# jaehyuck0103/OpenMAVIS

Measured on AMD Instinct MI355X. Metric: multi-cam frames/sec (ORB extract+match) + LocalBA iters/sec, 5x720x540, higher is better.
Workload: dtype u8

## Files before the change

openmavis_amd/csrc/omv_device.h:

```cpp
#pragma once
#include <hip/hip_runtime.h>
#include <stdint.h>

namespace omv {

__device__ __forceinline__ int round_even(float v) { return (int)__builtin_rintf(v); }

__device__ __forceinline__ float fast_atan2_deg(float y, float x) {
    const float r2d = (float)(180.0 / 3.14159265358979323846);
    const float k1 = 0.9997878412794807f * r2d;
    const float k3 = -0.3258083974640975f * r2d;
    const float k5 = 0.1555786518463281f * r2d;
    const float k7 = -0.04432655554792128f * r2d;
    const float eps = (float)2.220446049250313080847e-16;
    float ax = __builtin_fabsf(x), ay = __builtin_fabsf(y), a, c, c2;
    if (ax >= ay) {
        c = ay / (ax + eps);
        c2 = c * c;
        a = (((k7 * c2 + k5) * c2 + k3) * c2 + k1) * c;
    } else {
        c = ax / (ay + eps);
        c2 = c * c;
        a = 90.f - (((k7 * c2 + k5) * c2 + k3) * c2 + k1) * c;
    }
// ... 180 lines not shown
    w = x + r;
    if (ix >= 0x3f2ca140) {
        v = (float)iy;
        return (float)(1 - ((hx >> 30) & 2)) * (v - 2.0f * (x - (w * w / (w + v) - r)));
    }
    if (iy == 1) return w;
    float a, t;
    z = __uint_as_float(f32_bits(w) & 0xfffff000u);
    v = r - (z - x);
    t = a = -1.0f / w;
    t = __uint_as_float(f32_bits(t) & 0xfffff000u);
    s = 1.0f + t * z;
    return t + a * (s + t * v);
}
__device__ inline float glibc_tanf(float x) {
    const int32_t ix = (int32_t)(f32_bits(x) & 0x7fffffffu);
    if (ix <= 0x3f490fda) return glibc_kernel_tanf(x, 0.0f, 1);
    const double xd = (double)x, nd = rint(xd * 0.6366197723675814);
    const int n = (int)nd;
    const double r = xd - nd * 1.5707963267948966;
    const float y0 = (float)r, y1 = (float)(r - (double)y0);
    return glibc_kernel_tanf(y0, y1, 1 - ((n & 1) << 1));
}

__device__ __forceinline__ int xcd_block(int n_logical) {
    const int chunk = (n_logical + 7) >> 3;
    const int b = (int)(blockIdx.x & 7) * chunk + (int)(blockIdx.x >> 3);
    return b < n_logical ? b : -1;
}
__host__ inline int xcd_grid(int n_logical) { return (n_logical + 7) & ~7; }

}
extern "C" __device__ __attribute__((const)) uint32_t omv_llvm_mul_u24(uint32_t, uint32_t) __asm("llvm.amdgcn.mul.u24.i32");
namespace omv {
__device__ __forceinline__ int mul_u24(int a, int b) { return (int)omv_llvm_mul_u24((uint32_t)a, (uint32_t)b); }

struct MatcherKnobs {
    int bow_top = -1, tri_slices = -1, tri_ecap = -1, tri_walk_seq = 0;
    int cand_mode = 0;
    int cand_pw = -1;
};
MatcherKnobs matcher_knobs(const struct ::omv_matcher *m);
size_t matcher_kf_entry_cap(const struct ::omv_matcher *m);

}
```

openmavis_amd/csrc/orb_extract.hip:

```cpp
#include <hip/hip_runtime.h>

#include <algorithm>
#include <cmath>
#include <cstdlib>
#include <climits>
#include <cstdio>
#include <cstring>
#include <vector>

#include "../../include/omv.h"
#include "omv_device.h"
#include "omv_host.h"
#include "omv_introsort.h"

namespace {

constexpr int kMaxLevels = 16;
constexpr int kOrbStages = 4;
constexpr int kEdge = 19;
constexpr int kMinB = kEdge - 3;
#define OMV_PATTERN_TABLE_BEGIN
#define OMV_PATTERN_TABLE_END
constexpr int kPattern[256 * 4] = {
#include "orb_pattern_31.inc"
// ... 28 lines not shown
    int xq_off, use_xq;
    uint32_t m_quads, m_groups, m_w;
};

struct Cell {
    int level, y0, y1, x0, x1;
};

struct Geom {
    int nlevels;
    int W, H;
    int ini_th, min_th;
    int n_cells;
    int cell_cap;
    long long pyr_bytes;
    long long cand_per_img;
    int out_per_img;
    int n_max;
    int node_cap;
    int ccnt_cap;
    unsigned long long umax_pk;
    LevelGeom lv[kMaxLevels];
};

struct XTab {
    int sx0, sx1, coef;
};

struct __attribute__((aligned(16))) XQuad {
    int a[2];
    uint32_t sel[4], cf[4];
    int pad[2];
};
static_assert(sizeof(XQuad) == 48, "XQuad LDS addressing");

__device__ __forceinline__ const uint8_t *level_base(const Geom &g, const uint8_t *images, size_t img_stride,
                                                     size_t pitch0, const uint8_t *pyr, int img, int l,
                                                     int *pitch) {
    if (l == 0) {
        *pitch = (int)pitch0;
        return images + (size_t)img * img_stride;
    }
    *pitch = g.lv[l].pitch;
    return pyr + (size_t)img * g.pyr_bytes + g.lv[l].off;
}

constexpr int kPyrBlock = 16;

__device__ __forceinline__ int vmix(int b0, int b1, int h0, int h1) {
    return ((omv::mul_u24(b0, h0 >> 4) >> 16) + (omv::mul_u24(b1, h1 >> 4) >> 16) + 2) >> 2;
}

__global__ void __launch_bounds__(256) pyr_resize_kernel(Geom g, int l, const uint8_t *images, size_t img_stride,
                                                         size_t pitch0, uint8_t *pyr, const XTab *xt,
                                                         const XTab *yt, const XQuad *xq, int n_images) {
    extern __shared__ __attribute__((aligned(16))) uint32_t pyr_lds[];
    const LevelGeom &L = g.lv[l];
    const int img = blockIdx.y, tid = threadIdx.x;
    const int dy0 = blockIdx.x * kPyrBlock, dy1 = min(dy0 + kPyrBlock, L.h);
    int sp;
    const uint8_t *src = level_base(g, images, img_stride, pitch0, pyr, img, l - 1, &sp);
    const int sw = g.lv[l - 1].w;
    const int ndw = ((sw + 15) >> 4) << 2;
    const int nq = (L.w + 3) >> 2;
    XTab *xs = reinterpret_cast<XTab *>(pyr_lds);
    XQuad *xqs = reinterpret_cast<XQuad *>(pyr_lds);
    uint32_t *rows = pyr_lds + 12 * nq;
    const int sy0 = yt[L.ytab_off + dy0].sx0, sy1 = yt[L.ytab_off + dy1 - 1].sx1;
    const int nr = sy1 - sy0 + 1;
    XTab *ys = reinterpret_cast<XTab *>(rows + nr * ndw + 4);
    const bool quad = L.use_xq != 0;
    if (quad)
        for (int i = tid; i < nq; i += 256) xqs[i] = xq[L.xq_off + i];
    else
        for (int i = tid; i < L.w; i += 256) xs[i] = xt[L.xtab_off + i];
    if (tid < dy1 - dy0) ys[tid] = yt[L.ytab_off + dy0 + tid];
    if ((sp & 15) == 0 && (((uintptr_t)src) & 15) == 0) {
        const int n4 = ndw >> 2;
        const uint32_t m4 = g.lv[l - 1].m_groups;
        for (int q = tid; q < nr * n4; q += 256) {
            const int r = (int)__umulhi((uint32_t)q, m4), i = q - r * n4;
            reinterpret_cast<uint4 *>(rows)[q] = reinterpret_cast<const uint4 *>(src + (size_t)(sy0 + r) * sp)[i];
        }
    } else {
        uint8_t *b = reinterpret_cast<uint8_t *>(rows);
        const uint32_t mw = g.lv[l - 1].m_w;
        for (int q = tid; q < nr * sw; q += 256) {
            const int r = (int)__umulhi((uint32_t)q, mw), i = q - r * sw;
            b[(size_t)r * ndw * 4 + i] = src[(size_t)(sy0 + r) * sp + i];
        }
    }
    __syncthreads();
    const uint32_t mq = L.m_quads;
    typedef unsigned short u16x2 __attribute__((ext_vector_type(2)));
    for (int q = tid; q < (dy1 - dy0) * nq; q += 256) {
        const int r = (int)__umulhi((uint32_t)q, mq), qd = q - omv::mul_u24(r, nq), dx0 = qd * 4,
                  dy = dy0 + r;
        const XTab y = ys[r];
        const int b0 = (short)(y.coef & 0xffff), b1 = (short)(y.coef >> 16);
        uint32_t packed = 0;
        if (quad) {
            const XQuad X = *reinterpret_cast<const XQuad *>(reinterpret_cast<const char *>(xqs) + omv::mul_u24(qd, 48u));
            const uint32_t *R0 = rows + omv::mul_u24(y.sx0 - sy0, ndw),
                           *R1 = rows + omv::mul_u24(y.sx1 - sy0, ndw);
            const uint32_t u0[4] = {R0[X.a[0]], R0[X.a[0] + 1], R0[X.a[1]], R0[X.a[1] + 1]};
            const uint32_t u1[4] = {R1[X.a[0]], R1[X.a[0] + 1], R1[X.a[1]], R1[X.a[1] + 1]};
#pragma unroll
            for (int j = 0; j < 4; ++j) {
                const int pp = 2 * (j >> 1);
                const u16x2 cf = __builtin_bit_cast(u16x2, X.cf[j]);
                const int h0 = (int)__builtin_amdgcn_udot2(
                    __builtin_bit_cast(u16x2, __builtin_amdgcn_perm(u0[pp + 1], u0[pp], X.sel[j])), cf, 0u, false);
                const int h1 = (int)__builtin_amdgcn_udot2(
                    __builtin_bit_cast(u16x2, __builtin_amdgcn_perm(u1[pp + 1], u1[pp], X.sel[j])), cf, 0u, false);
                packed |= (uint32_t)vmix(b0, b1, h0, h1) << (8 * j);
            }
        } else {
            const uint8_t *R0 = reinterpret_cast<const uint8_t *>(rows + omv::mul_u24(y.sx0 - sy0, ndw));
            const uint8_t *R1 = reinterpret_cast<const uint8_t *>(rows + omv::mul_u24(y.sx1 - sy0, ndw));
#pragma unroll
            for (int j = 0; j < 4; ++j) {
                const int dx = dx0 + j;
                if (dx < L.w) {
                    const XTab x = xs[dx];
                    const int a0 = (short)(x.coef & 0xffff), a1 = (short)(x.coef >> 16);
                    const int h0 = R0[x.sx0] * a0 + R0[x.sx1] * a1;
                    const int h1 = R1[x.sx0] * a0 + R1[x.sx1] * a1;
                    const int v = vmix(b0, b1, h0, h1);
                    packed |= (uint32_t)min(v, 255) << (8 * j);
                }
            }
        }
        uint8_t *dst = pyr + (size_t)img * g.pyr_bytes + L.off + (size_t)dy * L.pitch;
        if (dx0 + 3 < L.w) {
            *reinterpret_cast<uint32_t *>(dst + dx0) = packed;
        } else {
            for (int j = 0; j < 4 && dx0 + j < L.w; ++j) dst[dx0 + j] = (uint8_t)(packed >> (8 * j));
        }
    }
}


struct PyrBand {
    int own_lo, own_hi, need_lo, need_hi;
};
constexpr int kPyrChainMaxImages = 16;
__global__ void __launch_bounds__(256) pyr_chain_kernel(Geom g, const uint8_t *images, size_t img_stride, size_t pitch0,
                                                        uint8_t *pyr, const XTab *xt, const XTab *yt, const XQuad *xq,
                                                        const PyrBand *bands, int buf_dw, int tab_dw) {
    extern __shared__ __attribute__((aligned(16))) uint32_t pyr_lds[];
    const int b = blockIdx.x, img = blockIdx.y, tid = threadIdx.x;
    const PyrBand *B = bands + (size_t)b * kMaxLevels;
    uint32_t *prev = pyr_lds, *cur = pyr_lds + buf_dw;
    uint32_t *tab = pyr_lds + 2 * (size_t)buf_dw + 4;
    XTab *ys = reinterpret_cast<XTab *>(tab + tab_dw);
    XQuad *xqs = reinterpret_cast<XQuad *>(tab);
    XTab *xs = reinterpret_cast<XTab *>(tab);
    {
        const PyrBand b0 = B[0];
        const int sw = g.lv[0].w, ndw = ((sw + 15) >> 4) << 2, nr = b0.need_hi - b0.need_lo;
        const uint8_t *src = images + (size_t)img * img_stride;
        if ((pitch0 & 15) == 0 && (((uintptr_t)src) & 15) == 0) {
            const int n4 = ndw >> 2;
            const uint32_t m4 = g.lv[0].m_groups;
            for (int q = tid; q < nr * n4; q += 256) {
                const int r = (int)__umulhi((uint32_t)q, m4), i = q - r * n4;
                reinterpret_cast<uint4 *>(prev)[q] = reinterpret_cast<const uint4 *>(src + (size_t)(b0.need_lo + r) * pitch0)[i];
            }
        } else {
            uint8_t *bb = reinterpret_cast<uint8_t *>(prev);
            const uint32_t mw = g.lv[0].m_w;
            for (int q = tid; q < nr * sw; q += 256) {
                const int r = (int)__umulhi((uint32_t)q, mw), i = q - r * sw;
                bb[(size_t)r * ndw * 4 + i] = src[(size_t)(b0.need_lo + r) * pitch0 + i];
            }
        }
    }
    __syncthreads();
    typedef unsigned short u16x2 __attribute__((ext_vector_type(2)));
    for (int l = 1; l < g.nlevels; ++l) {
        const LevelGeom &L = g.lv[l];
        const PyrBand bp = B[l - 1], bc = B[l];
        const int sndw = ((g.lv[l - 1].w + 15) >> 4) << 2, cndw = ((L.w + 15) >> 4) << 2;
        const int nq = (L.w + 3) >> 2, nr = bc.need_hi - bc.need_lo;
        const bool quad = L.use_xq != 0;
        if (quad)
            for (int i = tid; i < nq; i += 256) xqs[i] = xq[L.xq_off + i];
        else
            for (int i = tid; i < L.w; i += 256) xs[i] = xt[L.xtab_off + i];
        for (int i = tid; i < nr; i += 256) ys[i] = yt[L.ytab_off + bc.need_lo + i];
        __syncthreads();
        const uint32_t mq = L.m_quads;
        for (int q = tid; q < nr * nq; q += 256) {
            const int r = (int)__umulhi((uint32_t)q, mq), qd = q - omv::mul_u24(r, nq), dx0 = qd * 4,
                      dy = bc.need_lo + r;
            const XTab y = ys[r];
            const int b0 = (short)(y.coef & 0xffff), b1 = (short)(y.coef >> 16);
            uint32_t packed = 0;
            if (quad) {
                const XQuad X = *reinterpret_cast<const XQuad *>(reinterpret_cast<const char *>(xqs) + omv::mul_u24(qd, 48u));
                const uint32_t *R0 = prev + omv::mul_u24(y.sx0 - bp.need_lo, sndw),
                               *R1 = prev + omv::mul_u24(y.sx1 - bp.need_lo, sndw);
                const uint32_t u0[4] = {R0[X.a[0]], R0[X.a[0] + 1], R0[X.a[1]], R0[X.a[1] + 1]};
                const uint32_t u1[4] = {R1[X.a[0]], R1[X.a[0] + 1], R1[X.a[1]], R1[X.a[1] + 1]};
#pragma unroll
                for (int j = 0; j < 4; ++j) {
                    const int pp = 2 * (j >> 1);
                    const u16x2 cf = __builtin_bit_cast(u16x2, X.cf[j]);
                    const int h0 = (int)__builtin_amdgcn_udot2(
                        __builtin_bit_cast(u16x2, __builtin_amdgcn_perm(u0[pp + 1], u0[pp], X.sel[j])), cf, 0u, false);
                    const int h1 = (int)__builtin_amdgcn_udot2(
                        __builtin_bit_cast(u16x2, __builtin_amdgcn_perm(u1[pp + 1], u1[pp], X.sel[j])), cf, 0u, false);
                    packed |= (uint32_t)vmix(b0, b1, h0, h1) << (8 * j);
                }
            } else {
                const uint8_t *R0 = reinterpret_cast<const uint8_t *>(prev + omv::mul_u24(y.sx0 - bp.need_lo, sndw));
                const uint8_t *R1 = reinterpret_cast<const uint8_t *>(prev + omv::mul_u24(y.sx1 - bp.need_lo, sndw));
#pragma unroll
                for (int j = 0; j < 4; ++j) {
                    const int dx = dx0 + j;
                    if (dx < L.w) {
                        const XTab x = xs[dx];
                        const int a0 = (short)(x.coef & 0xffff), a1 = (short)(x.coef >> 16);
                        const int h0 = R0[x.sx0] * a0 + R0[x.sx1] * a1;
                        const int h1 = R1[x.sx0] * a0 + R1[x.sx1] * a1;
                        const int v = vmix(b0, b1, h0, h1);
                        packed |= (uint32_t)min(v, 255) << (8 * j);
                    }
                }
            }
            cur[omv::mul_u24(r, cndw) + qd] = packed;
            if (dy >= bc.own_lo && dy < bc.own_hi) {
                uint8_t *dst = pyr + (size_t)img * g.pyr_bytes + L.off + (size_t)dy * L.pitch;
                if (dx0 + 3 < L.w) {
                    *reinterpret_cast<uint32_t *>(dst + dx0) = packed;
                } else {
                    for (int j = 0; j < 4 && dx0 + j < L.w; ++j) dst[dx0 + j] = (uint8_t)(packed >> (8 * j));
                }
            }
        }
        __syncthreads();
        uint32_t *t = prev;
        prev = cur, cur = t;
    }
}

typedef short pk16 __attribute__((ext_vector_type(2)));

typedef _Float16 h2 __attribute__((ext_vector_type(2)));
__device__ __forceinline__ h2 h2_swap(h2 x) { return h2{x.y, x.x}; }
typedef unsigned short u16x2 __attribute__((ext_vector_type(2)));
__device__ __forceinline__ h2 h2_biased(const uint8_t *lo, const uint8_t *hi) {
    const u16x2 v{(unsigned short)*lo, (unsigned short)*hi};
    return __builtin_bit_cast(h2, __builtin_bit_cast(uint32_t, v) | 0x64006400u);
}

template <int RS>
__device__ __forceinline__ int fast_strength_h(const uint8_t *p, int stride_rt) {
    const int stride = RS > 0 ? RS : stride_rt;
    const int o[16] = {3 * stride, 3 * stride + 1, 2 * stride + 2, stride + 3, 3, -stride + 3, -2 * stride + 2,
                       -3 * stride + 1, -3 * stride, -3 * stride - 1, -2 * stride - 2, -stride - 3, -3, stride - 3,
                       2 * stride - 2, 3 * stride - 1};
    const h2 vv = h2_biased(p, p);
    h2 d[8];
#pragma unroll
    for (int k = 0; k < 8; ++k) d[k] = vv - h2_biased(p + o[k], p + o[k + 8]);
    auto Q = [&](const h2 *a, int k) { return k < 8 ? a[k] : h2_swap(a[k - 8]); };
    h2 t3n[8], t3x[8];
#pragma unroll
    for (int k = 0; k < 8; ++k) {
        t3n[k] = __builtin_elementwise_minimum(__builtin_elementwise_minimum(d[k], Q(d, k + 1)), Q(d, k + 2));
// ... 873 lines not shown
    omv::block_introsort_loop(items, n, stk, LS, RS, threadIdx.x, blockDim.x);
    omv::block_final_insertion_sort(items, n, tmp, threadIdx.x, blockDim.x);
    for (int i = threadIdx.x; i < n; i += blockDim.x) perm[i] = items[i].payload;
}

}

struct omv_orb {
    omv_orb_params p;
    int W, H, max_images;
    int pyr_mode = -1;
    std::vector<float> scale, inv_scale, sigma2, inv_sigma2;
    std::vector<int> quota;
    int umax[16];
    Geom g;
    Cell *d_cells = nullptr;
    XTab *d_xt = nullptr, *d_yt = nullptr;
    XQuad *d_xq = nullptr;
    uint32_t *d_disc = nullptr;
    float *harris = nullptr;
    uint8_t *d_pyr = nullptr;
    int *d_cell_cnt = nullptr;
    uint32_t *d_cell_kp = nullptr, *d_cand = nullptr, *d_nid = nullptr, *d_lvl_out = nullptr, *d_lvl_cls = nullptr;
    int *d_lvl_cnt = nullptr, *d_lap = nullptr, *d_err = nullptr;
    int rmax = 0;
    int smax = 0;
    int fast_rs = 0;
    size_t fast_lds = 0;
    size_t oct_lds = 0;
    size_t pyr_lds[kMaxLevels] = {};
    PyrBand *d_bands = nullptr;
    int pyr_nb = 0, pyr_buf_dw = 0;
    int pyr_tab_dw = 0, pyr_rows = 0;
    uint8_t *d_img1 = nullptr;
    omv_kp *d_kp1 = nullptr;
    uint8_t *d_desc1 = nullptr;
    int *d_n1 = nullptr;
    std::vector<int> h_lap;
    hipStream_t last_stream = nullptr;
    int last_n = 0;
    int device = 0;
    bool timing = false;
    std::vector<hipEvent_t> ev;
    double stage_ms[kOrbStages] = {};
    long long stage_calls = 0;
};

static void flush_timing(omv_orb *o) {
    for (size_t b = 0; b + kOrbStages + 1 <= o->ev.size(); b += kOrbStages + 1) {
        for (int k = 0; k < kOrbStages; ++k) {
            float ms = 0.f;
            (void)hipEventElapsedTime(&ms, o->ev[b + k], o->ev[b + k + 1]);
            o->stage_ms[k] += ms;
        }
        o->stage_calls++;
    }
    for (hipEvent_t e : o->ev) (void)hipEventDestroy(e);
    o->ev.clear();
}

static void mark(omv_orb *o, hipStream_t st) {
    if (!o->timing) return;
    hipEvent_t e;
    (void)hipEventCreate(&e);
    (void)hipEventRecord(e, st);
    o->ev.push_back(e);
// ... 86 lines not shown
            const int sw = prev_w, sh = prev_h, dw = L.w, dh = L.h;
            L.xtab_off = (int)xt.size();
            L.ytab_off = (int)yt.size();
            const double sx_scale = 1.0 / ((double)dw / sw), sy_scale = 1.0 / ((double)dh / sh);
            int xmax = dw;
            std::vector<XTab> row(dw);
            for (int dx = 0; dx < dw; ++dx) {
                float fx = (float)((dx + 0.5) * sx_scale - 0.5);
                int sx = (int)std::floor(fx);
                fx -= sx;
                if (sx < 0) fx = 0, sx = 0;
                if (sx + 1 >= sw) {
                    xmax = std::min(xmax, dx);
                    if (sx >= sw - 1) fx = 0, sx = sw - 1;
                }
                int a0 = (short)host_round_even((1.f - fx) * 2048.f), a1 = (short)host_round_even(fx * 2048.f);
                row[dx] = XTab{sx, std::min(sx + 1, sw - 1), (a0 & 0xffff) | (a1 << 16)};
            }
            for (int dx = xmax; dx < dw; ++dx) row[dx].coef = 2048, row[dx].sx1 = row[dx].sx0;
            xt.insert(xt.end(), row.begin(), row.end());
            L.xq_off = (int)xq.size();
            L.use_xq = 1;
            for (int q = 0; q < (dw + 3) / 4; ++q) {
                XQuad X{};
                for (int p = 0; p < 2; ++p) X.a[p] = (row[std::min(4 * q + 2 * p, dw - 1)].sx0) >> 2;
                for (int j = 0; j < 4; ++j) {
                    const int dx = 4 * q + j;
                    if (dx >= dw) {
                        X.sel[j] = 0x0c0c0c0cu, X.cf[j] = 0;
                        continue;
                    }
                    const int base = 4 * X.a[j >> 1], o0 = row[dx].sx0 - base, o1 = row[dx].sx1 - base;
                    const int a0 = (short)(row[dx].coef & 0xffff), a1 = (short)(row[dx].coef >> 16);
                    if (o0 < 0 || o0 > 7 || o1 < 0 || o1 > 7 || a0 < 0 || a1 < 0) L.use_xq = 0;
                    X.sel[j] = (uint32_t)(o0 & 7) | 0x0c00u | ((uint32_t)(o1 & 7) << 16) | 0x0c000000u;
                    X.cf[j] = (uint32_t)(a0 & 0xffff) | ((uint32_t)(a1 & 0xffff) << 16);
                }
                xq.push_back(X);
            }
            for (int dy = 0; dy < dh; ++dy) {
                float fy = (float)((dy + 0.5) * sy_scale - 0.5);
                int sy = (int)std::floor(fy);
                fy -= sy;
                int b0 = (short)host_round_even((1.f - fy) * 2048.f), b1 = (short)host_round_even(fy * 2048.f);
                const int r0 = std::min(std::max(sy, 0), sh - 1), r1 = std::min(std::max(sy + 1, 0), sh - 1);
                yt.push_back(XTab{r0, r1, (b0 & 0xffff) | (b1 << 16)});
            }
        }
        prev_w = L.w, prev_h = L.h;
        auto divm = [](int d) { return (uint32_t)((0x100000000ull + (uint64_t)d - 1) / (uint64_t)d); };
        L.m_quads = divm((L.w + 3) / 4), L.m_groups = divm((L.w + 15) / 16), L.m_w = divm(L.w);
    }
    g.n_cells = (int)cells.size();
    if (max_rw > 80 || max_rh > 80) return OMV_ERR_ARG;
    const int dw = max_rw - 6, dh = max_rh - 6;
    g.cell_cap = ((dw + 1) / 2) * ((dh + 1) / 2);
    for (int l = 0; l < nl; ++l) {
        LevelGeom &L = g.lv[l];
        L.cand_off = cand_off;
        L.cand_cap = (L.cell_end - L.cell_begin) * g.cell_cap;
        cand_off += L.cand_cap;
    }
    g.pyr_bytes = (pyr_off + 255) & ~255LL;
    g.cand_per_img = cand_off;
    g.out_per_img = out_off;
    g.n_max = out_off;
    g.node_cap = (max_nodes + 15) & ~15;
    g.ccnt_cap = (std::max(4 * g.node_cap, max_cells_lvl) + 15) & ~15;
    o->fast_rs = max_rw + 3 <= 52 ? 52 : max_rw + 3 <= 68 ? 68 : 0;
    if (const char *e = getenv("OMV_FAST_RS"))
        if (std::atoi(e) == 68 && max_rw + 3 <= 68) o->fast_rs = 68;
    o->rmax = ((o->fast_rs ? o->fast_rs * max_rh : ((max_rw + 6) & ~3) * max_rh) + 15) & ~15;
    o->smax = ((std::max(0, (max_rw - 4) * (max_rh - 4))) + 15) & ~15;
    o->fast_lds = (size_t)o->rmax + o->smax + 2 * (size_t)std::max(0, (max_rw - 6) * (max_rh - 6));
    o->oct_lds = (size_t)(32 + 14 * g.node_cap + g.ccnt_cap + 6 * (g.node_cap / 17 + 1) + 2) * sizeof(int);
    return OMV_OK;
}

// ... 26 lines not shown
    if (const char *pm = getenv("OMV_PYR_MODE")) o->pyr_mode = std::strcmp(pm, "chain") == 0 ? 1 : 0;
    (void)hipGetDevice(&o->device);
    std::vector<Cell> cells;
    std::vector<XTab> xt, yt;
    std::vector<XQuad> xq;
    omv_status st = build_geometry(o, cells, xt, yt, xq);
    if (st != OMV_OK) {
        delete o;
        return st;
    }
    if (o->oct_lds > 160 * 1024) {
        delete o;
        return OMV_ERR_ARG;
    }
    if (o->oct_lds > 64 * 1024 &&
        (hipFuncSetAttribute((const void *)octree_kernel<OMV_OCT_WGS>, hipFuncAttributeMaxDynamicSharedMemorySize,
                             (int)o->oct_lds) != hipSuccess ||
         hipFuncSetAttribute((const void *)octree_kernel<1>, hipFuncAttributeMaxDynamicSharedMemorySize,
                             (int)o->oct_lds) != hipSuccess)) {
        delete o;
        return OMV_ERR_HIP;
    }
    const Geom &g = o->g;
    const size_t n = (size_t)max_images;
    HIP_OK(hipMalloc(&o->d_cells, sizeof(Cell) * cells.size()));
    HIP_OK(hipMemcpy(o->d_cells, cells.data(), sizeof(Cell) * cells.size(), hipMemcpyHostToDevice));
    for (int l = 1; l < g.nlevels; ++l) {
        const LevelGeom &L = g.lv[l];
        int nr = 0;
        for (int dy0 = 0; dy0 < L.h; dy0 += kPyrBlock) {
            const int dy1 = std::min(dy0 + kPyrBlock, L.h);
            nr = std::max(nr, yt[L.ytab_off + dy1 - 1].sx1 - yt[L.ytab_off + dy0].sx0 + 1);
        }
        o->pyr_lds[l] = sizeof(uint32_t) * (12 * (size_t)((L.w + 3) / 4) + (size_t)nr * (((g.lv[l - 1].w + 15) / 16) * 4) + 4 +
                                            3 * kPyrBlock);
        if (o->pyr_lds[l] > 160 * 1024) {
            delete o;
            return OMV_ERR_ARG;
        }
        if (o->pyr_lds[l] > 64 * 1024)
            (void)hipFuncSetAttribute((const void *)pyr_resize_kernel, hipFuncAttributeMaxDynamicSharedMemorySize,
                                      (int)o->pyr_lds[l]);
    }
    {
        const int L = g.nlevels;
        auto plan = [&](int nb, std::vector<PyrBand> &bands) {
            bands.assign((size_t)nb * kMaxLevels, PyrBand{0, 0, 0, 0});
            int worst = 0;
            for (int b = 0; b < nb; ++b) {
                PyrBand *B = &bands[(size_t)b * kMaxLevels];
                for (int l = 1; l < L; ++l)
                    B[l].own_lo = (int)((long long)b * g.lv[l].h / nb), B[l].own_hi = (int)((long long)(b + 1) * g.lv[l].h / nb);
                B[L - 1].need_lo = B[L - 1].own_lo, B[L - 1].need_hi = B[L - 1].own_hi;
                for (int l = L - 1; l >= 1; --l) {
                    int lo = INT_MAX, hi = INT_MIN;
                    if (B[l].need_hi > B[l].need_lo)
                        lo = yt[g.lv[l].ytab_off + B[l].need_lo].sx0, hi = yt[g.lv[l].ytab_off + B[l].need_hi - 1].sx1 + 1;
                    if (l - 1 >= 1 && B[l - 1].own_hi > B[l - 1].own_lo)
                        lo = std::min(lo, B[l - 1].own_lo), hi = std::max(hi, B[l - 1].own_hi);
                    if (hi > lo) B[l - 1].need_lo = std::max(0, lo), B[l - 1].need_hi = std::min(g.lv[l - 1].h, hi);
                }
                for (int l = 0; l < L; ++l)
                    worst = std::max(worst, (B[l].need_hi - B[l].need_lo) * (((g.lv[l].w + 15) / 16) * 4));
            }
            return worst;
        };
        std::vector<PyrBand> bands;
        for (int budget : {8192, 16384}) {
            for (int nb = 8; nb <= 128 && L > 1 && !o->pyr_nb; ++nb) {
                const int worst = plan(nb, bands);
                if (worst > budget) continue;
                int tab = 0, rows = 0;
                for (int l = 1; l < L; ++l) {
                    tab = std::max(tab, g.lv[l].use_xq ? 12 * ((g.lv[l].w + 3) / 4) : 3 * g.lv[l].w);
                    for (int b = 0; b < nb; ++b) {
                        const PyrBand &pb = bands[(size_t)b * kMaxLevels + l];
                        rows = std::max(rows, pb.need_hi - pb.need_lo);
                    }
                }
                o->pyr_nb = nb, o->pyr_buf_dw = worst, o->pyr_tab_dw = (tab + 3) & ~3, o->pyr_rows = rows;
                HIP_OK(hipMalloc(&o->d_bands, sizeof(PyrBand) * bands.size()));
                HIP_OK(hipMemcpy(o->d_bands, bands.data(), sizeof(PyrBand) * bands.size(), hipMemcpyHostToDevice));
                const int lds = (int)(sizeof(uint32_t) * (2 * (size_t)worst + 4 + o->pyr_tab_dw + 3 * (size_t)rows));
                if (lds > 160 * 1024) {
                    (void)hipFree(o->d_bands);
                    o->d_bands = nullptr, o->pyr_nb = 0;
                    break;
                }
                if (lds > 64 * 1024)
                    (void)hipFuncSetAttribute((const void *)pyr_chain_kernel, hipFuncAttributeMaxDynamicSharedMemorySize, lds);
            }
        }
    }
    HIP_OK(hipMalloc(&o->d_xt, sizeof(XTab) * std::max<size_t>(1, xt.size())));
    HIP_OK(hipMalloc(&o->d_yt, sizeof(XTab) * std::max<size_t>(1, yt.size())));
    if (!xt.empty()) HIP_OK(hipMemcpy(o->d_xt, xt.data(), sizeof(XTab) * xt.size(), hipMemcpyHostToDevice));
    if (!yt.empty()) HIP_OK(hipMemcpy(o->d_yt, yt.data(), sizeof(XTab) * yt.size(), hipMemcpyHostToDevice));
    HIP_OK(hipMalloc(&o->d_xq, sizeof(XQuad) * std::max<size_t>(1, xq.size())));
    if (!xq.empty()) HIP_OK(hipMemcpy(o->d_xq, xq.data(), sizeof(XQuad) * xq.size(), hipMemcpyHostToDevice));
    {
        const std::vector<uint32_t> dt = disc_table(o->umax);
        HIP_OK(hipMalloc(&o->d_disc, sizeof(uint32_t) * dt.size()));
        HIP_OK(hipMemcpy(o->d_disc, dt.data(), sizeof(uint32_t) * dt.size(), hipMemcpyHostToDevice));
    }
    HIP_OK(hipMalloc(&o->d_pyr, std::max<size_t>(256, (size_t)g.pyr_bytes * n)));
    HIP_OK(hipMalloc(&o->d_cell_cnt, sizeof(int) * g.n_cells * n));
    HIP_OK(hipMalloc(&o->d_cell_kp, sizeof(uint32_t) * (size_t)g.n_cells * g.cell_cap * n));
    HIP_OK(hipMalloc(&o->d_cand, sizeof(uint32_t) * (size_t)g.cand_per_img * n));
    HIP_OK(hipMalloc(&o->d_nid, sizeof(uint32_t) * (size_t)g.cand_per_img * n));
    HIP_OK(hipMalloc(&o->d_lvl_out, sizeof(uint32_t) * (size_t)g.out_per_img * n));
    HIP_OK(hipMalloc(&o->d_lvl_cls, sizeof(uint32_t) * (size_t)g.out_per_img * n));
    HIP_OK(hipMalloc(&o->d_lvl_cnt, sizeof(int) * 3 * g.nlevels * n));
    HIP_OK(hipMalloc(&o->d_lap, sizeof(int) * 2 * n));
    HIP_OK(hipMalloc(&o->d_err, sizeof(int)));
    HIP_OK(hipMemset(o->d_err, 0, sizeof(int)));
    *out = o;
// ... 12 lines not shown
    return OMV_OK;
}

int omv_orb_max_keypoints(const omv_orb *o) { return o ? o->g.n_max : 0; }

omv_status omv_orb_scale_tables(const omv_orb *o, float *scale, float *inv_scale, float *sigma2, float *inv_sigma2) {
    if (!o) return OMV_ERR_ARG;
    for (int l = 0; l < o->p.nlevels; ++l) {
        if (scale) scale[l] = o->scale[l];
        if (inv_scale) inv_scale[l] = o->inv_scale[l];
        if (sigma2) sigma2[l] = o->sigma2[l];
        if (inv_sigma2) inv_sigma2[l] = o->inv_sigma2[l];
    }
    return OMV_OK;
}

omv_status omv_orb_extract_batch(omv_orb *o, int n, const uint8_t *images, size_t image_stride, size_t pitch,
                                 const int *lapping, omv_kp *kps, uint8_t *desc, int *n_out, int *mono_index,
                                 void *stream) {
    if (!o || n <= 0 || n > o->max_images || !images || !lapping || !kps || !desc || !n_out || !mono_index)
        return OMV_ERR_ARG;
    if (pitch < (size_t)o->W || image_stride < pitch * o->H) return OMV_ERR_ARG;
    hipStream_t st = (hipStream_t)stream;
    o->last_stream = st;
    o->last_n = n;
    const Geom &g = o->g;
    if (o->h_lap.size() < (size_t)2 * n || std::memcmp(o->h_lap.data(), lapping, sizeof(int) * 2 * n) != 0) {
        HIP_OK(hipMemcpyAsync(o->d_lap, lapping, sizeof(int) * 2 * n, hipMemcpyHostToDevice, st));
        o->h_lap.assign(lapping, lapping + 2 * n);
    }
    mark(o, st);
    const bool chain = o->pyr_mode >= 0 ? o->pyr_mode == 1 : n <= kPyrChainMaxImages;
    if (o->pyr_nb > 0 && chain) {
        const size_t lds = sizeof(uint32_t) * (2 * (size_t)o->pyr_buf_dw + 4 + o->pyr_tab_dw + 3 * (size_t)o->pyr_rows);
        pyr_chain_kernel<<<dim3(o->pyr_nb, n), 256, lds, st>>>(g, images, image_stride, pitch, o->d_pyr, o->d_xt, o->d_yt,
                                                               o->d_xq, o->d_bands, o->pyr_buf_dw, o->pyr_tab_dw);
    } else {
        for (int l = 1; l < g.nlevels; ++l) {
            pyr_resize_kernel<<<dim3((g.lv[l].h + kPyrBlock - 1) / kPyrBlock, n), 256, o->pyr_lds[l], st>>>(
                g, l, images, image_stride, pitch, o->d_pyr, o->d_xt, o->d_yt, o->d_xq, n);
        }
    }
    mark(o, st);
    if (o->fast_rs == 52)
        fast_cells_kernel<52><<<omv::xcd_grid(g.n_cells * n), 64, o->fast_lds, st>>>(
            g, o->d_cells, images, image_stride, pitch, o->d_pyr, o->d_cell_cnt, o->d_cell_kp, o->rmax, o->smax,
            g.n_cells * n);
    else if (o->fast_rs == 68)
        fast_cells_kernel<68><<<omv::xcd_grid(g.n_cells * n), 64, o->fast_lds, st>>>(
            g, o->d_cells, images, image_stride, pitch, o->d_pyr, o->d_cell_cnt, o->d_cell_kp, o->rmax, o->smax,
            g.n_cells * n);
    else
        fast_cells_kernel<0><<<omv::xcd_grid(g.n_cells * n), 64, o->fast_lds, st>>>(
            g, o->d_cells, images, image_stride, pitch, o->d_pyr, o->d_cell_cnt, o->d_cell_kp, o->rmax, o->smax,
            g.n_cells * n);
    mark(o, st);
    OctArgs oa{o->d_cell_cnt, o->d_cell_kp, o->d_cand, o->d_nid, o->d_lvl_out, o->d_lvl_cls, o->d_lvl_cnt, o->d_lap, o->d_err};
    if (n <= kOctSmallImages) octree_kernel<1><<<g.nlevels * n, 256, o->oct_lds, st>>>(g, oa);
    else octree_kernel<OMV_OCT_WGS><<<g.nlevels * n, 256, o->oct_lds, st>>>(g, oa);
    mark(o, st);
    DescArgs da{images, image_stride, pitch, o->d_pyr, o->d_lvl_out, o->d_lvl_cls, o->d_lvl_cnt, kps, desc, n_out, mono_index, n,
                o->d_disc, o->harris};
    const int waves = g.out_per_img * n;
    describe_kernel<<<omv::xcd_grid((waves + 3) / 4), 256, 0, st>>>(g, da, (waves + 3) / 4);
    mark(o, st);
    HIP_OK(hipGetLastError());
    return OMV_OK;
// ... 102 lines not shown
```

Before: 44240.

## Process pyramid resize in vertical strips reusing horizontal sums across rows

The pyramid resize and chain kernels now give each thread a column quad over a strip of 8 output rows. It computes the horizontal interpolation sums once per source row and reuses them when consecutive output rows share a source row, instead of recomputing per output pixel. XQuad coefficients are held in registers, loaded straight from global memory, rather than staged in LDS. The LDS footprint is capped at a hold size to raise occupancy. Row staging now issues four 16-byte loads per iteration before storing, and pre-scaled coefficients with a mulhi_u24 vertical blend replace the old mix; these add host-side range checks, and exact rounding must match the previous path.

```diff
diff --git a/openmavis_amd/csrc/omv_device.h b/openmavis_amd/csrc/omv_device.h
--- a/openmavis_amd/csrc/omv_device.h
+++ b/openmavis_amd/csrc/omv_device.h
@@ -236,8 +236,10 @@
 
 }
 extern "C" __device__ __attribute__((const)) uint32_t omv_llvm_mul_u24(uint32_t, uint32_t) __asm("llvm.amdgcn.mul.u24.i32");
+extern "C" __device__ __attribute__((const)) uint32_t omv_llvm_mulhi_u24(uint32_t, uint32_t) __asm("llvm.amdgcn.mulhi.u24");
 namespace omv {
 __device__ __forceinline__ int mul_u24(int a, int b) { return (int)omv_llvm_mul_u24((uint32_t)a, (uint32_t)b); }
+__device__ __forceinline__ uint32_t mulhi_u24(uint32_t a, uint32_t b) { return omv_llvm_mulhi_u24(a, b); }
 
 struct MatcherKnobs {
     int bow_top = -1, tri_slices = -1, tri_ecap = -1, tri_walk_seq = 0;
diff --git a/openmavis_amd/csrc/orb_extract.hip b/openmavis_amd/csrc/orb_extract.hip
--- a/openmavis_amd/csrc/orb_extract.hip
+++ b/openmavis_amd/csrc/orb_extract.hip
@@ -84,7 +84,12 @@
     uint32_t sel[4], cf[4];
     int pad[2];
 };
-static_assert(sizeof(XQuad) == 48, "XQuad LDS addressing");
+static_assert(sizeof(XQuad) == 48, "XQuad: three 16-byte loads");
+
+struct __attribute__((aligned(16))) YRow {
+    int o0, o1;
+    uint32_t b0, b1;
+};
 
 __device__ __forceinline__ const uint8_t *level_base(const Geom &g, const uint8_t *images, size_t img_stride,
                                                      size_t pitch0, const uint8_t *pyr, int img, int l,
@@ -98,9 +103,84 @@
 }
 
 constexpr int kPyrBlock = 16;
+constexpr size_t kPyrLdsHold = 24 * 1024;
 
 __device__ __forceinline__ int vmix(int b0, int b1, int h0, int h1) {
     return ((omv::mul_u24(b0, h0 >> 4) >> 16) + (omv::mul_u24(b1, h1 >> 4) >> 16) + 2) >> 2;
+}
+
+constexpr int kPyrStrip = 8;
+
+__device__ __forceinline__ void pyr_hsums(uint32_t h[4], const XQuad &X, const char *c0, const char *c1, int o) {
+    typedef unsigned short u16x2 __attribute__((ext_vector_type(2)));
+    const uint32_t *p0 = reinterpret_cast<const uint32_t *>(c0 + o), *p1 = reinterpret_cast<const uint32_t *>(c1 + o);
+    const uint32_t u[4] = {p0[0], p0[1], p1[0], p1[1]};
+#pragma unroll
+    for (int j = 0; j < 4; ++j) {
+        const int pp = 2 * (j >> 1);
+        h[j] = __builtin_amdgcn_udot2(__builtin_bit_cast(u16x2, __builtin_amdgcn_perm(u[pp + 1], u[pp], X.sel[j])),
+                                      __builtin_bit_cast(u16x2, X.cf[j]), 0u, false) & 0xffffff00u;
+    }
+}
+
+template <class Emit>
+__device__ __forceinline__ void pyr_strip(const XQuad &X, const uint32_t *rows, const YRow *ys, int n, Emit emit) {
+    const char *c0 = reinterpret_cast<const char *>(rows + X.a[0]), *c1 = reinterpret_cast<const char *>(rows + X.a[1]);
+    uint32_t hA[4], hB[4];
+    int idA = -1, idB = -1;
+    for (int r = 0; r < n; ++r) {
+        const YRow y = ys[r];
+        if (y.o0 != idA) {
+            if (y.o0 == idB) {
+#pragma unroll
+                for (int j = 0; j < 4; ++j) hA[j] = hB[j];
+            } else {
+                pyr_hsums(hA, X, c0, c1, y.o0);
+            }
+            idA = y.o0;
+        }
+        if (y.o1 != idB) {
+            pyr_hsums(hB, X, c0, c1, y.o1);
+            idB = y.o1;
+        }
+        uint32_t packed = 0;
+#pragma unroll
+        for (int j = 0; j < 4; ++j)
+            packed |= ((omv::mulhi_u24(y.b0, hA[j]) + omv::mulhi_u24(y.b1, hB[j]) + 2) >> 2) << (8 * j);
+        emit(packed);
+    }
+}
+
+__device__ __forceinline__ void pyr_stage16(uint32_t *rows, const uint8_t *src, size_t sp, int nr, int n4, uint32_t m4,
+                                            int tid) {
+    const int total = nr * n4;
+    for (int q = tid; q < total; q += 4 * 256) {
+        uint4 v[4];
+#pragma unroll
+        for (int k = 0; k < 4; ++k) {
+            const int qk = min(q + 256 * k, total - 1);
+            const int r = (int)__umulhi((uint32_t)qk, m4), i = qk - r * n4;
+            v[k] = reinterpret_cast<const uint4 *>(src + (size_t)r * sp)[i];
+        }
+#pragma unroll
+        for (int k = 0; k < 4; ++k)
+            if (q + 256 * k < total) reinterpret_cast<uint4 *>(rows)[q + 256 * k] = v[k];
+    }
+}
+
+__device__ __forceinline__ YRow pyr_yrow(const XTab y, int sbase, int ndw) {
+    return YRow{omv::mul_u24(y.sx0 - sbase, ndw) * 4, omv::mul_u24(y.sx1 - sbase, ndw) * 4,
+                ((uint32_t)y.coef & 0xffffu) << 8, ((uint32_t)y.coef >> 16) << 8};
+}
+
+__device__ __forceinline__ void pyr_store(uint8_t *dst, uint32_t packed, int left) {
+    if (left >= 4) {
+        *reinterpret_cast<uint32_t *>(dst) = packed;
+    } else {
+#pragma unroll
+        for (int j = 0; j < 3; ++j)
+            if (j < left) dst[j] = (uint8_t)(packed >> (8 * j));
+    }
 }
 
 __global__ void __launch_bounds__(256) pyr_resize_kernel(Geom g, int l, const uint8_t *images, size_t img_stride,
@@ -115,25 +195,27 @@
     const int sw = g.lv[l - 1].w;
     const int ndw = ((sw + 15) >> 4) << 2;
     const int nq = (L.w + 3) >> 2;
+    const bool quad = L.use_xq != 0;
     XTab *xs = reinterpret_cast<XTab *>(pyr_lds);
-    XQuad *xqs = reinterpret_cast<XQuad *>(pyr_lds);
-    uint32_t *rows = pyr_lds + 12 * nq;
+    uint32_t *rows = pyr_lds + (quad ? 0 : 12 * nq);
     const int sy0 = yt[L.ytab_off + dy0].sx0, sy1 = yt[L.ytab_off + dy1 - 1].sx1;
     const int nr = sy1 - sy0 + 1;
+    const int nt = quad ? ((dy1 - dy0 + kPyrStrip - 1) / kPyrStrip) * nq : 0;
+    const uint32_t mq = L.m_quads;
+    int s = (int)__umulhi((uint32_t)tid, mq), qd = tid - omv::mul_u24(s, nq);
+    XQuad X{};
+    if (tid < nt) X = xq[L.xq_off + qd];
     XTab *ys = reinterpret_cast<XTab *>(rows + nr * ndw + 4);
-    const bool quad = L.use_xq != 0;
-    if (quad)
-        for (int i = tid; i < nq; i += 256) xqs[i] = xq[L.xq_off + i];
-    else
+    YRow *ysq = reinterpret_cast<YRow *>(rows + nr * ndw + 4);
+    if (!quad)
         for (int i = tid; i < L.w; i += 256) xs[i] = xt[L.xtab_off + i];
-    if (tid < dy1 - dy0) ys[tid] = yt[L.ytab_off + dy0 + tid];
+    if (tid < dy1 - dy0) {
+        const XTab y = yt[L.ytab_off + dy0 + tid];
+        if (quad) ysq[tid] = pyr_yrow(y, sy0, ndw);
+        else ys[tid] = y;
+    }
     if ((sp & 15) == 0 && (((uintptr_t)src) & 15) == 0) {
-        const int n4 = ndw >> 2;
-        const uint32_t m4 = g.lv[l - 1].m_groups;
-        for (int q = tid; q < nr * n4; q += 256) {
-            const int r = (int)__umulhi((uint32_t)q, m4), i = q - r * n4;
-            reinterpret_cast<uint4 *>(rows)[q] = reinterpret_cast<const uint4 *>(src + (size_t)(sy0 + r) * sp)[i];
-        }
+        pyr_stage16(rows, src + (size_t)sy0 * sp, (size_t)sp, nr, ndw >> 2, g.lv[l - 1].m_groups, tid);
     } else {
         uint8_t *b = reinterpret_cast<uint8_t *>(rows);
         const uint32_t mw = g.lv[l - 1].m_w;
@@ -143,52 +225,42 @@
         }
     }
     __syncthreads();
-    const uint32_t mq = L.m_quads;
-    typedef unsigned short u16x2 __attribute__((ext_vector_type(2)));
+    uint8_t *out = pyr + (size_t)img * g.pyr_bytes + L.off + (size_t)dy0 * L.pitch;
+    if (quad) {
+        for (int t = tid; t < nt; t += 256) {
+            if (t != tid) {
+                s = (int)__umulhi((uint32_t)t, mq), qd = t - omv::mul_u24(s, nq);
+                X = xq[L.xq_off + qd];
+            }
+            const int r0 = s * kPyrStrip, left = L.w - 4 * qd, pitch = L.pitch;
+            uint8_t *dst = out + (size_t)omv::mul_u24(r0, pitch) + 4 * qd;
+            pyr_strip(X, rows, ysq + r0, min(kPyrStrip, dy1 - dy0 - r0), [&](uint32_t packed) {
+                pyr_store(dst, packed, left);
+                dst += pitch;
+            });
+        }
+        return;
+    }
     for (int q = tid; q < (dy1 - dy0) * nq; q += 256) {
-        const int r = (int)__umulhi((uint32_t)q, mq), qd = q - omv::mul_u24(r, nq), dx0 = qd * 4,
-                  dy = dy0 + r;
+        const int r = (int)__umulhi((uint32_t)q, mq), qd = q - omv::mul_u24(r, nq), dx0 = qd * 4;
         const XTab y = ys[r];
         const int b0 = (short)(y.coef & 0xffff), b1 = (short)(y.coef >> 16);
         uint32_t packed = 0;
-        if (quad) {
-            const XQuad X = *reinterpret_cast<const XQuad *>(reinterpret_cast<const char *>(xqs) + omv::mul_u24(qd, 48u));
-            const uint32_t *R0 = rows + omv::mul_u24(y.sx0 - sy0, ndw),
-                           *R1 = rows + omv::mul_u24(y.sx1 - sy0, ndw);
-            const uint32_t u0[4] = {R0[X.a[0]], R0[X.a[0] + 1], R0[X.a[1]], R0[X.a[1] + 1]};
-            const uint32_t u1[4] = {R1[X.a[0]], R1[X.a[0] + 1], R1[X.a[1]], R1[X.a[1] + 1]};
-#pragma unroll
-            for (int j = 0; j < 4; ++j) {
-                const int pp = 2 * (j >> 1);
-                const u16x2 cf = __builtin_bit_cast(u16x2, X.cf[j]);
-                const int h0 = (int)__builtin_amdgcn_udot2(
-                    __builtin_bit_cast(u16x2, __builtin_amdgcn_perm(u0[pp + 1], u0[pp], X.sel[j])), cf, 0u, false);
-                const int h1 = (int)__builtin_amdgcn_udot2(
-                    __builtin_bit_cast(u16x2, __builtin_amdgcn_perm(u1[pp + 1], u1[pp], X.sel[j])), cf, 0u, false);
-                packed |= (uint32_t)vmix(b0, b1, h0, h1) << (8 * j);
-            }
-        } else {
-            const uint8_t *R0 = reinterpret_cast<const uint8_t *>(rows + omv::mul_u24(y.sx0 - sy0, ndw));
-            const uint8_t *R1 = reinterpret_cast<const uint8_t *>(rows + omv::mul_u24(y.sx1 - sy0, ndw));
-#pragma unroll
-            for (int j = 0; j < 4; ++j) {
-                const int dx = dx0 + j;
-                if (dx < L.w) {
-                    const XTab x = xs[dx];
-                    const int a0 = (short)(x.coef & 0xffff), a1 = (short)(x.coef >> 16);
-                    const int h0 = R0[x.sx0] * a0 + R0[x.sx1] * a1;
-                    const int h1 = R1[x.sx0] * a0 + R1[x.sx1] * a1;
-                    const int v = vmix(b0, b1, h0, h1);
-                    packed |= (uint32_t)min(v, 255) << (8 * j);
-                }
-            }
-        }
-        uint8_t *dst = pyr + (size_t)img * g.pyr_bytes + L.off + (size_t)dy * L.pitch;
-        if (dx0 + 3 < L.w) {
-            *reinterpret_cast<uint32_t *>(dst + dx0) = packed;
-        } else {
-            for (int j = 0; j < 4 && dx0 + j < L.w; ++j) dst[dx0 + j] = (uint8_t)(packed >> (8 * j));
-        }
+        const uint8_t *R0 = reinterpret_cast<const uint8_t *>(rows + omv::mul_u24(y.sx0 - sy0, ndw));
+        const uint8_t *R1 = reinterpret_cast<const uint8_t *>(rows + omv::mul_u24(y.sx1 - sy0, ndw));
+#pragma unroll
+        for (int j = 0; j < 4; ++j) {
+            const int dx = dx0 + j;
+            if (dx < L.w) {
+                const XTab x = xs[dx];
+                const int a0 = (short)(x.coef & 0xffff), a1 = (short)(x.coef >> 16);
+                const int h0 = R0[x.sx0] * a0 + R0[x.sx1] * a1;
+                const int h1 = R1[x.sx0] * a0 + R1[x.sx1] * a1;
+                const int v = vmix(b0, b1, h0, h1);
+                packed |= (uint32_t)min(v, 255) << (8 * j);
+            }
+        }
+        pyr_store(out + (size_t)r * L.pitch + dx0, packed, L.w - dx0);
     }
 }
 
@@ -206,19 +278,14 @@
     uint32_t *prev = pyr_lds, *cur = pyr_lds + buf_dw;
     uint32_t *tab = pyr_lds + 2 * (size_t)buf_dw + 4;
     XTab *ys = reinterpret_cast<XTab *>(tab + tab_dw);
-    XQuad *xqs = reinterpret_cast<XQuad *>(tab);
+    YRow *ysq = reinterpret_cast<YRow *>(tab + tab_dw);
     XTab *xs = reinterpret_cast<XTab *>(tab);
     {
         const PyrBand b0 = B[0];
         const int sw = g.lv[0].w, ndw = ((sw + 15) >> 4) << 2, nr = b0.need_hi - b0.need_lo;
         const uint8_t *src = images + (size_t)img * img_stride;
         if ((pitch0 & 15) == 0 && (((uintptr_t)src) & 15) == 0) {
-            const int n4 = ndw >> 2;
-            const uint32_t m4 = g.lv[0].m_groups;
-            for (int q = tid; q < nr * n4; q += 256) {
-                const int r = (int)__umulhi((uint32_t)q, m4), i = q - r * n4;
-                reinterpret_cast<uint4 *>(prev)[q] = reinterpret_cast<const uint4 *>(src + (size_t)(b0.need_lo + r) * pitch0)[i];
-            }
+            pyr_stage16(prev, src + (size_t)b0.need_lo * pitch0, pitch0, nr, ndw >> 2, g.lv[0].m_groups, tid);
         } else {
             uint8_t *bb = reinterpret_cast<uint8_t *>(prev);
             const uint32_t mw = g.lv[0].m_w;
@@ -229,43 +296,44 @@
         }
     }
     __syncthreads();
-    typedef unsigned short u16x2 __attribute__((ext_vector_type(2)));
     for (int l = 1; l < g.nlevels; ++l) {
         const LevelGeom &L = g.lv[l];
         const PyrBand bp = B[l - 1], bc = B[l];
         const int sndw = ((g.lv[l - 1].w + 15) >> 4) << 2, cndw = ((L.w + 15) >> 4) << 2;
         const int nq = (L.w + 3) >> 2, nr = bc.need_hi - bc.need_lo;
         const bool quad = L.use_xq != 0;
-        if (quad)
-            for (int i = tid; i < nq; i += 256) xqs[i] = xq[L.xq_off + i];
-        else
+        if (!quad)
             for (int i = tid; i < L.w; i += 256) xs[i] = xt[L.xtab_off + i];
-        for (int i = tid; i < nr; i += 256) ys[i] = yt[L.ytab_off + bc.need_lo + i];
+        for (int i = tid; i < nr; i += 256) {
+            const XTab y = yt[L.ytab_off + bc.need_lo + i];
+            if (quad) ysq[i] = pyr_yrow(y, bp.need_lo, sndw);
+            else ys[i] = y;
+        }
         __syncthreads();
         const uint32_t mq = L.m_quads;
-        for (int q = tid; q < nr * nq; q += 256) {
-            const int r = (int)__umulhi((uint32_t)q, mq), qd = q - omv::mul_u24(r, nq), dx0 = qd * 4,
-                      dy = bc.need_lo + r;
-            const XTab y = ys[r];
-            const int b0 = (short)(y.coef & 0xffff), b1 = (short)(y.coef >> 16);
-            uint32_t packed = 0;
-            if (quad) {
-                const XQuad X = *reinterpret_cast<const XQuad *>(reinterpret_cast<const char *>(xqs) + omv::mul_u24(qd, 48u));
-                const uint32_t *R0 = prev + omv::mul_u24(y.sx0 - bp.need_lo, sndw),
-                               *R1 = prev + omv::mul_u24(y.sx1 - bp.need_lo, sndw);
-                const uint32_t u0[4] = {R0[X.a[0]], R0[X.a[0] + 1], R0[X.a[1]], R0[X.a[1] + 1]};
-                const uint32_t u1[4] = {R1[X.a[0]], R1[X.a[0] + 1], R1[X.a[1]], R1[X.a[1] + 1]};
-#pragma unroll
-                for (int j = 0; j < 4; ++j) {
-                    const int pp = 2 * (j >> 1);
-                    const u16x2 cf = __builtin_bit_cast(u16x2, X.cf[j]);
-                    const int h0 = (int)__builtin_amdgcn_udot2(
-                        __builtin_bit_cast(u16x2, __builtin_amdgcn_perm(u0[pp + 1], u0[pp], X.sel[j])), cf, 0u, false);
-                    const int h1 = (int)__builtin_amdgcn_udot2(
-                        __builtin_bit_cast(u16x2, __builtin_amdgcn_perm(u1[pp + 1], u1[pp], X.sel[j])), cf, 0u, false);
-                    packed |= (uint32_t)vmix(b0, b1, h0, h1) << (8 * j);
-                }
-            } else {
+        uint8_t *out = pyr + (size_t)img * g.pyr_bytes + L.off;
+        if (quad) {
+            const int ns = (nr + kPyrStrip - 1) / kPyrStrip;
+            for (int t = tid; t < ns * nq; t += 256) {
+                const int s = (int)__umulhi((uint32_t)t, mq), qd = t - omv::mul_u24(s, nq), r0 = s * kPyrStrip;
+                const XQuad X = xq[L.xq_off + qd];
+                const int left = L.w - 4 * qd, pitch = L.pitch;
+                int dy = bc.need_lo + r0;
+                uint32_t *c = cur + omv::mul_u24(r0, cndw) + qd;
+                uint8_t *dst = out + (size_t)dy * pitch + 4 * qd;
+                pyr_strip(X, prev, ysq + r0, min(kPyrStrip, nr - r0), [&](uint32_t packed) {
+                    *c = packed;
+                    if (dy >= bc.own_lo && dy < bc.own_hi) pyr_store(dst, packed, left);
+                    c += cndw, dst += pitch, ++dy;
+                });
+            }
+        } else {
+            for (int q = tid; q < nr * nq; q += 256) {
+                const int r = (int)__umulhi((uint32_t)q, mq), qd = q - omv::mul_u24(r, nq), dx0 = qd * 4,
+                          dy = bc.need_lo + r;
+                const XTab y = ys[r];
+                const int b0 = (short)(y.coef & 0xffff), b1 = (short)(y.coef >> 16);
+                uint32_t packed = 0;
                 const uint8_t *R0 = reinterpret_cast<const uint8_t *>(prev + omv::mul_u24(y.sx0 - bp.need_lo, sndw));
                 const uint8_t *R1 = reinterpret_cast<const uint8_t *>(prev + omv::mul_u24(y.sx1 - bp.need_lo, sndw));
 #pragma unroll
@@ -280,15 +348,9 @@
                         packed |= (uint32_t)min(v, 255) << (8 * j);
                     }
                 }
-            }
-            cur[omv::mul_u24(r, cndw) + qd] = packed;
-            if (dy >= bc.own_lo && dy < bc.own_hi) {
-                uint8_t *dst = pyr + (size_t)img * g.pyr_bytes + L.off + (size_t)dy * L.pitch;
-                if (dx0 + 3 < L.w) {
-                    *reinterpret_cast<uint32_t *>(dst + dx0) = packed;
-                } else {
-                    for (int j = 0; j < 4 && dx0 + j < L.w; ++j) dst[dx0 + j] = (uint8_t)(packed >> (8 * j));
-                }
+                cur[omv::mul_u24(r, cndw) + qd] = packed;
+                if (dy >= bc.own_lo && dy < bc.own_hi)
+                    pyr_store(out + (size_t)dy * L.pitch + dx0, packed, L.w - dx0);
             }
         }
         __syncthreads();
@@ -1228,6 +1290,7 @@
     PyrBand *d_bands = nullptr;
     int pyr_nb = 0, pyr_buf_dw = 0;
     int pyr_tab_dw = 0, pyr_rows = 0;
+    int pyr_ydw = 3;
     uint8_t *d_img1 = nullptr;
     omv_kp *d_kp1 = nullptr;
     uint8_t *d_desc1 = nullptr;
@@ -1380,9 +1443,9 @@
                     }
                     const int base = 4 * X.a[j >> 1], o0 = row[dx].sx0 - base, o1 = row[dx].sx1 - base;
                     const int a0 = (short)(row[dx].coef & 0xffff), a1 = (short)(row[dx].coef >> 16);
-                    if (o0 < 0 || o0 > 7 || o1 < 0 || o1 > 7 || a0 < 0 || a1 < 0) L.use_xq = 0;
+                    if (o0 < 0 || o0 > 7 || o1 < 0 || o1 > 7 || a0 < 0 || a1 < 0 || a0 > 2048 || a1 > 2048) L.use_xq = 0;
                     X.sel[j] = (uint32_t)(o0 & 7) | 0x0c00u | ((uint32_t)(o1 & 7) << 16) | 0x0c000000u;
-                    X.cf[j] = (uint32_t)(a0 & 0xffff) | ((uint32_t)(a1 & 0xffff) << 16);
+                    X.cf[j] = (uint32_t)((16 * a0) & 0xffff) | ((uint32_t)((16 * a1) & 0xffff) << 16);
                 }
                 xq.push_back(X);
             }
@@ -1392,6 +1455,7 @@
                 fy -= sy;
                 int b0 = (short)host_round_even((1.f - fy) * 2048.f), b1 = (short)host_round_even(fy * 2048.f);
                 const int r0 = std::min(std::max(sy, 0), sh - 1), r1 = std::min(std::max(sy + 1, 0), sh - 1);
+                if (b0 < 0 || b1 < 0 || b0 > 2048 || b1 > 2048) L.use_xq = 0;
                 yt.push_back(XTab{r0, r1, (b0 & 0xffff) | (b1 << 16)});
             }
         }
@@ -1484,8 +1548,12 @@
             const int dy1 = std::min(dy0 + kPyrBlock, L.h);
             nr = std::max(nr, yt[L.ytab_off + dy1 - 1].sx1 - yt[L.ytab_off + dy0].sx0 + 1);
         }
-        o->pyr_lds[l] = sizeof(uint32_t) * (12 * (size_t)((L.w + 3) / 4) + (size_t)nr * (((g.lv[l - 1].w + 15) / 16) * 4) + 4 +
-                                            3 * kPyrBlock);
+        const size_t rows_dw = (size_t)nr * (((g.lv[l - 1].w + 15) / 16) * 4) + 4;
+        o->pyr_lds[l] = sizeof(uint32_t) * (12 * (size_t)((L.w + 3) / 4) + rows_dw + 3 * kPyrBlock);
+        if (L.use_xq) {
+            const size_t need = sizeof(uint32_t) * (rows_dw + 4 * kPyrBlock);
+            o->pyr_lds[l] = std::max(need, std::min(o->pyr_lds[l], kPyrLdsHold));
+        }
         if (o->pyr_lds[l] > 160 * 1024) {
             delete o;
             return OMV_ERR_ARG;
@@ -1522,18 +1590,19 @@
             for (int nb = 8; nb <= 128 && L > 1 && !o->pyr_nb; ++nb) {
                 const int worst = plan(nb, bands);
                 if (worst > budget) continue;
-                int tab = 0, rows = 0;
+                int tab = 0, rows = 0, ydw = 3;
                 for (int l = 1; l < L; ++l) {
-                    tab = std::max(tab, g.lv[l].use_xq ? 12 * ((g.lv[l].w + 3) / 4) : 3 * g.lv[l].w);
+                    if (g.lv[l].use_xq) ydw = 4;
+                    else tab = std::max(tab, 3 * g.lv[l].w);
                     for (int b = 0; b < nb; ++b) {
                         const PyrBand &pb = bands[(size_t)b * kMaxLevels + l];
                         rows = std::max(rows, pb.need_hi - pb.need_lo);
                     }
                 }
-                o->pyr_nb = nb, o->pyr_buf_dw = worst, o->pyr_tab_dw = (tab + 3) & ~3, o->pyr_rows = rows;
+                o->pyr_nb = nb, o->pyr_buf_dw = worst, o->pyr_tab_dw = (tab + 3) & ~3, o->pyr_rows = rows, o->pyr_ydw = ydw;
                 HIP_OK(hipMalloc(&o->d_bands, sizeof(PyrBand) * bands.size()));
                 HIP_OK(hipMemcpy(o->d_bands, bands.data(), sizeof(PyrBand) * bands.size(), hipMemcpyHostToDevice));
-                const int lds = (int)(sizeof(uint32_t) * (2 * (size_t)worst + 4 + o->pyr_tab_dw + 3 * (size_t)rows));
+                const int lds = (int)(sizeof(uint32_t) * (2 * (size_t)worst + 4 + o->pyr_tab_dw + (size_t)ydw * rows));
                 if (lds > 160 * 1024) {
                     (void)hipFree(o->d_bands);
                     o->d_bands = nullptr, o->pyr_nb = 0;
@@ -1612,7 +1681,7 @@
     mark(o, st);
     const bool chain = o->pyr_mode >= 0 ? o->pyr_mode == 1 : n <= kPyrChainMaxImages;
     if (o->pyr_nb > 0 && chain) {
-        const size_t lds = sizeof(uint32_t) * (2 * (size_t)o->pyr_buf_dw + 4 + o->pyr_tab_dw + 3 * (size_t)o->pyr_rows);
+        const size_t lds = sizeof(uint32_t) * (2 * (size_t)o->pyr_buf_dw + 4 + o->pyr_tab_dw + (size_t)o->pyr_ydw * o->pyr_rows);
         pyr_chain_kernel<<<dim3(o->pyr_nb, n), 256, lds, st>>>(g, images, image_stride, pitch, o->d_pyr, o->d_xt, o->d_yt,
                                                                o->d_xq, o->d_bands, o->pyr_buf_dw, o->pyr_tab_dw);
     } else {
```

Result: faster. 45110 (median of 6 runs) (+2.0%).
